# apache/bifromq

Hardware: AMD Instinct MI355X
Metric: publish-topic matches/sec (whole node) (higher is better)
Workload: dtype u32

## Files before the change

### bifromq_amd/csrc/bmq_build_core.h

```cpp
#pragma once
#include <sched.h>
#include <stdint.h>

#include "bmq_layout.h"

namespace bmq {

#if defined(__HIP_DEVICE_COMPILE__)
#define BMQ_MO_LOAD __ATOMIC_RELAXED
#define BMQ_MO_STORE __ATOMIC_RELAXED
#define BMQ_MO_RMW __ATOMIC_RELAXED
template <class T> BMQ_HD T atom_load(const T* p) { return __hip_atomic_load(p, __ATOMIC_RELAXED, __HIP_MEMORY_SCOPE_AGENT); }
template <class T> BMQ_HD void shared_store(T* p, T v) { __hip_atomic_store(p, v, __ATOMIC_RELAXED, __HIP_MEMORY_SCOPE_AGENT); }
template <class T> BMQ_HD T shared_load(const T* p) { return __hip_atomic_load(p, __ATOMIC_RELAXED, __HIP_MEMORY_SCOPE_AGENT); }
template <class T> BMQ_HD void atom_publish(T* p, T v) {
    asm volatile("s_waitcnt vmcnt(0)" ::: "memory");
    __hip_atomic_store(p, v, __ATOMIC_RELAXED, __HIP_MEMORY_SCOPE_AGENT);
}
template <class T> BMQ_HD T atom_cas(T* p, T expect, T desired) {
    __hip_atomic_compare_exchange_strong(p, &expect, desired, __ATOMIC_RELAXED, __ATOMIC_RELAXED, __HIP_MEMORY_SCOPE_AGENT);
    return expect;
}
template <class T> BMQ_HD T atom_add(T* p, T v) { return __hip_atomic_fetch_add(p, v, __ATOMIC_RELAXED, __HIP_MEMORY_SCOPE_AGENT); }
template <class T> BMQ_HD T atom_or(T* p, T v) { return __hip_atomic_fetch_or(p, v, __ATOMIC_RELAXED, __HIP_MEMORY_SCOPE_AGENT); }
// ... 181 lines not shown
}
BMQ_HD uint32_t tail_hash(const uint8_t* kp, unsigned long long beg, unsigned long long end) {
    uint32_t h = 0x811C9DC5u ^ (uint32_t)(end - beg);
    for (unsigned long long p = beg; p < end; p += 16) {
        uint32_t w[4];
        bytes_chunk16(kp, p, (uint32_t)(end - p < 16 ? end - p : 16), w);
        h = (h ^ w[0]) * 0x01000193u;
        h = (rotl32(h, 13) ^ w[1]) * 0x01000193u;
        h = (rotl32(h, 13) ^ w[2]) * 0x01000193u;
        h = (rotl32(h, 13) ^ w[3]) * 0x01000193u;
    }
    return mix32(h) | 1u;
}
BMQ_HD bool pool_bytes_equal(const uint8_t* kp, unsigned long long ao, unsigned long long bo, unsigned long long n) {
    for (unsigned long long i = 0; i < n; i += 16) {
        uint32_t x[4], y[4];
        const uint32_t m = (uint32_t)(n - i < 16 ? n - i : 16);
        bytes_chunk16(kp, ao + i, m, x);
        bytes_chunk16(kp, bo + i, m, y);
        if (((x[0] ^ y[0]) | (x[1] ^ y[1]) | (x[2] ^ y[2]) | (x[3] ^ y[3])) != 0) return false;
    }
    return true;
}
BMQ_HD bool bytes_equal(const uint8_t* a, unsigned long long ao, const uint8_t* b, unsigned long long bo, unsigned long long n) {
    for (unsigned long long i = 0; i < n; i++)
        if (a[ao + i] != b[bo + i]) return false;
    return true;
}
BMQ_HD int bytes_compare(const uint8_t* p, unsigned long long a, unsigned long long an, unsigned long long b, unsigned long long bn) {
    const unsigned long long m = an < bn ? an : bn;
    for (unsigned long long i = 0; i < m; i++) {
        const int d = (int)p[a + i] - (int)p[b + i];
        if (d) return d;
    }
    return an < bn ? -1 : (an > bn ? 1 : 0);
}

BMQ_HD uint32_t tenant_find(const TenantSlot* dir, uint32_t mask, const uint8_t* names, const uint8_t* kp, unsigned long long beg,
                            unsigned long long end) {
    const uint64_t h = tenant_hash_bytes(kp, beg, end);
    const uint32_t lo = (uint32_t)h, hi = (uint32_t)(h >> 32), len = (uint32_t)(end - beg);
    uint32_t d = (lo ^ hi) & mask;
    for (uint32_t probes = 0; probes <= mask; probes++) {
        const TenantSlot& t = dir[d];
        if (t.hash_lo == 0 && t.hash_hi == 0) return NONE;
        if (t.hash_lo == lo && t.hash_hi == hi && t.name_len == len && bytes_equal(names, t.name_off, kp, beg, len)) return d;
        d = (d + 1) & mask;
    }
    return NONE;
}

BMQ_HD uint32_t dict_intern(const DistIndexMut& ix, const LevelHash& h, uint32_t len, const uint32_t inl[4], const uint8_t* kp,
                            unsigned long long start, bool insert) {
    const uint32_t tag = level_hash_tag(h);
    uint32_t g = level_hash_slot(h, len) & ix.dict_group_mask;
    for (uint32_t jj = 0; jj < DICT_GROUP; jj++) {
        const DictSlot* s = ix.dict + DICT_GROUP * (size_t)g + jj;
        if (peek_load(&s->tag) != tag) continue;
        const uint32_t tok = peek_load(&s->token);
        if (tok == 0 || peek_load(&s->len) != len || peek_load(&s->inl[0]) != inl[0] || peek_load(&s->inl[1]) != inl[1] || peek_load(&s->inl[2]) != inl[2] ||
            peek_load(&s->inl[3]) != inl[3])
            continue;
        bool eq = true;
        if (len > 16) {
            const uint32_t po = peek_load(&s->pool_off);
            for (uint32_t i = 16; i < len && eq; i++) eq = peek_load(ix.dpool + po + i) == kp[start + i];
        }
        if (eq) return tok;
    }
    uint32_t j = 0, probes = 0, spins = 0;
    const uint32_t max_probes = insert && ix.dict_group_mask > 128u ? 128u : ix.dict_group_mask;
    for (;;) {
        if (probes > max_probes || spins > (1u << 22)) {
            atom_or(&ix.bc->err, probes > max_probes ? (uint32_t)ERR_DICT_FULL : (uint32_t)ERR_STUCK);
            return TOK_UNKNOWN;
        }
        DictSlot* s = ix.dict + DICT_GROUP * (size_t)g + j;
        uint32_t t = atom_load(&s->tag);
        if (t == 0) {
            if (!insert) return TOK_UNKNOWN;
            t = atom_cas(&s->tag, 0u, tag);
            if (t == 0) {
                uint32_t off = 0;
                if (len > 16) {
                    off = atom_add(&ix.bc->dpool_used, (len + 3u) & ~3u);
                    if ((unsigned long long)off + len > ix.dpool_cap) {
                        atom_or(&ix.bc->err, (uint32_t)ERR_DICT_FULL);
                        off = 0;
                    } else
                        for (uint32_t i = 0; i < len; i++) shared_store(ix.dpool + off + i, kp[start + i]);
                }
                shared_store(&s->len, len);
                shared_store(&s->pool_off, off);
                shared_store(&s->inl[0], inl[0]);
                shared_store(&s->inl[1], inl[1]);
                shared_store(&s->inl[2], inl[2]);
                shared_store(&s->inl[3], inl[3]);
                const uint32_t tok = TOK_FIRST + atom_add(&ix.bc->n_tokens, 1u);
                atom_publish(&s->token, tok);
                return tok;
            }
        }
        if (t == tag) {
            const uint32_t tok = atom_load(&s->token);
            if (tok == 0) {
                spin_pause(spins++);
                continue;
            }
            bool eq = shared_load(&s->len) == len && shared_load(&s->inl[0]) == inl[0] && shared_load(&s->inl[1]) == inl[1] &&
                      shared_load(&s->inl[2]) == inl[2] && shared_load(&s->inl[3]) == inl[3];
            if (eq && len > 16) {
                const uint32_t po = shared_load(&s->pool_off);
                for (uint32_t i = 16; i < len && eq; i++) eq = shared_load(ix.dpool + po + i) == kp[start + i];
            }
            if (eq) return tok;
        }
        if (++j == DICT_GROUP) {
            j = 0;
            g = (g + 1) & ix.dict_group_mask;
            probes++;
        }
    }
}

constexpr unsigned long long PARENT_IS_ROOT = ~0ull;
BMQ_HD uint32_t trie_child(const DistIndexMut& ix, TenantSlot* ten, uint32_t base, uint32_t buckets, uint32_t parent, unsigned long long parent_slot,
                           uint32_t token, bool insert, unsigned long long& slot_abs, bool& created) {
    created = false;
    const uint64_t key = (uint64_t)parent | ((uint64_t)token << 32);
    const bool root_plus = token == TOK_PLUS && parent_slot == PARENT_IS_ROOT;
    const bool try_beside = token == TOK_PLUS && parent_slot != PARENT_IS_ROOT;
    const unsigned long long beside_abs = parent_slot ^ 1ull;
    uint32_t phase = 0, spins = 0, bk = 0, j = 0, probes = 0;
    TrieSlot* wait = nullptr;
    unsigned long long wait_abs = 0;
    {
        auto peek = [&](unsigned long long abs) -> uint32_t {
            const TrieSlot* s = ix.trie + (size_t)abs;
            if (peek_load(reinterpret_cast<const uint64_t*>(s)) != key) return NONE;
            return peek_load(&s->node);
        };
        if (try_beside) {
            const uint32_t id = peek(beside_abs);
            if (id != NONE) {
                slot_abs = beside_abs;
                return id;
            }
        }
        if (!root_plus) {
            const unsigned long long home = (unsigned long long)base + 2ull * edge_bucket(parent, token, buckets);
            for (uint32_t jj = 0; jj < 2; jj++) {
                const uint32_t id = peek(home + jj);
                if (id != NONE) {
                    slot_abs = home + jj;
                    return id;
                }
            }
        }
    }
    for (;;) {
        if (spins > (1u << 22)) {
            atom_or(&ix.bc->err, (uint32_t)ERR_STUCK);
            return NONE;
// ... 566 lines not shown
            rec.parent = x.node;
            rec.token = TOK_TAIL;
            rec.own_begin = c.own_count != 0 ? c.own_begin : c.hash_begin;
            rec.own_count = c.own_count != 0 ? c.own_count : (c.hash_count | TAIL_HASH);
            rec.hash_begin = toks[0], rec.hash_count = toks[1], rec.node = toks[2], rec.lit_bloom = toks[3];
            ix.trie[g ^ 1u] = rec;
            return;
        }
        if (n != 1u || c.own_count != 0 || c.hash_count != 0) return;
        rel = tp.kid[r->nbase + c.node];
    }
}


BMQ_HD bool find_filter(const DistIndexMut& ix, const uint8_t* q, uint32_t tenant_len, uint32_t filter_len, IdSet& out) {
    out = IdSet{0, 0};
    const uint32_t d = tenant_find(ix.tenants, ix.tenant_mask, ix.tenant_names, q, 0, tenant_len);
    if (d == NONE) return false;
    TenantSlot* ten = ix.tenants + d;
    uint32_t node = 0;
    unsigned long long slot_abs = 0, pos = tenant_len;
    const unsigned long long end = (unsigned long long)tenant_len + filter_len;
    bool at_root = true;
    for (;;) {
        LevelHash h;
        uint32_t inl[4], len;
        const unsigned long long start = pos;
        scan_level_bytes<0x2F2F2F2Fu>(q, pos, end, h, inl, len);
        const bool last = pos >= end;
        if (level_is_hash(q, start, len, last)) {
            if (at_root) out = IdSet{ten->root_hash_begin, ten->root_hash_count};
            else out = IdSet{ix.trie[slot_abs].hash_begin, ix.trie[slot_abs].hash_count};
            return out.count() != 0;
        }
        const uint32_t tok = level_is_plus(q, start, len) ? TOK_PLUS : dict_intern(ix, h, len, inl, q, start, false);
        if (tok == TOK_UNKNOWN) return false;
        bool created;
        node = trie_child(ix, ten, ten->base, ten->buckets, node, at_root ? PARENT_IS_ROOT : slot_abs, tok, false, slot_abs, created);
        if (node == NONE) return false;
        at_root = false;
        if (last) break;
        pos++;
    }
    out = IdSet{ix.trie[slot_abs].own_begin, ix.trie[slot_abs].own_count};
    return out.count() != 0;
}

BMQ_HD void dict_rehash_one(const DictSlot* old, uint32_t i, const DistIndexMut& ix) {
    const DictSlot s = old[i];
    if (s.tag == 0) return;
    LevelHash h = level_hash_init();
    for (uint32_t o = 0; o < s.len; o += 4) {
        uint32_t w;
        if (s.len <= 16) w = s.inl[o >> 2];
        else {
            w = 0;
            for (uint32_t k = 0; k < 4 && o + k < s.len; k++) w |= (uint32_t)ix.dpool[s.pool_off + o + k] << (8 * k);
        }
        level_hash_word(h, w);
    }
    uint32_t g = level_hash_slot(h, s.len) & ix.dict_group_mask, j = 0;
    for (uint32_t probes = 0; probes <= ix.dict_group_mask;) {
        DictSlot* d = ix.dict + DICT_GROUP * (size_t)g + j;
        if (atom_cas(&d->tag, 0u, s.tag) == 0u) {
            d->len = s.len;
            d->pool_off = s.pool_off;
            d->inl[0] = s.inl[0];
            d->inl[1] = s.inl[1];
            d->inl[2] = s.inl[2];
            d->inl[3] = s.inl[3];
            d->token = s.token;
            return;
        }
        if (++j == DICT_GROUP) {
            j = 0;
            g = (g + 1) & ix.dict_group_mask;
            probes++;
        }
    }
    atom_or(&ix.bc->err, (uint32_t)ERR_DICT_FULL);
}

BMQ_HD void find_copy(const DistIndexMut& ix, const uint8_t* q, uint32_t tenant_len, uint32_t filter_len, uint32_t* out, uint32_t cap) {
    IdSet s;
    if (!find_filter(ix, q, tenant_len, filter_len, s)) {
        out[0] = 0;
        return;
    }
    const uint32_t n = s.count();
    out[0] = n;
    for (uint32_t m = 0; m < n && m < cap; m++) out[1 + m] = idset_at(ix, s, m);
}
BMQ_HD void gather_ref_one(const DistIndexMut& ix, const uint32_t* ids, uint32_t i, uint32_t id_end, unsigned long long* out) {
    const uint32_t id = ids[i];
    out[i] = id < id_end && id < ix.id_cap ? ix.kref[id] : 0ull;
}
BMQ_HD void gather_bytes_one(const DistIndexMut& ix, const unsigned long long* refs, const uint64_t* offs, uint32_t i, uint8_t* out) {
    const unsigned long long r = refs[i];
    const unsigned long long off = r & KREF_OFF_MASK, len = r >> KREF_LEN_SHIFT;
    for (unsigned long long k = 0; k < len; k++) out[offs[i] + k] = ix.kpool[off + k];
}

struct KeyBoundary {
    const uint8_t* start;
    const uint8_t* end;
    uint32_t start_len, end_len;
    uint32_t flags;
};
BMQ_HD int key_compare(const uint8_t* a, unsigned long long an, const uint8_t* b, unsigned long long bn) {
    const unsigned long long m = an < bn ? an : bn;
    unsigned long long p = 0;
    for (; p + 8 <= m; p += 8) {
        unsigned long long x, y;
        __builtin_memcpy(&x, a + p, 8);
        __builtin_memcpy(&y, b + p, 8);
        if (x != y) return __builtin_bswap64(x) < __builtin_bswap64(y) ? -1 : 1;
    }
    for (; p < m; p++)
        if (a[p] != b[p]) return a[p] < b[p] ? -1 : 1;
    return an < bn ? -1 : (an > bn ? 1 : 0);
}
BMQ_HD bool key_in_boundary(const uint8_t* kpool, unsigned long long ref, const KeyBoundary& b) {
    const uint8_t* k = kpool + (ref & KREF_OFF_MASK);
// ... 25 lines not shown
```

### bifromq_amd/csrc/bmq_dict.h

```cpp
#pragma once
#include <algorithm>
#include <cstring>
#include <string_view>
#include <vector>

#include "bmq_layout.h"

namespace bmq {

inline LevelHash hash_level(std::string_view s) {
    LevelHash h = level_hash_init();
    for (size_t i = 0; i < s.size(); i += 4) {
        uint32_t w = 0;
        for (size_t k = 0; k < 4 && i + k < s.size(); k++) w |= (uint32_t)(uint8_t)s[i + k] << (8 * k);
        level_hash_word(h, w);
    }
    return h;
}

inline uint32_t pow2_at_least(uint64_t v) {
    uint32_t p = 64;
    while (p < v && p < 0x80000000u) p <<= 1;
    return p;
}

struct HostDict {
    struct Entry {
        std::string_view s;
        uint32_t slot_hash, tag;
    };
    std::vector<Entry> entries;
    std::vector<uint32_t> table;
    uint32_t mask = 0;
    HostDict() { table.assign(1024, 0); mask = 1023; }
    void grow() {
        std::vector<uint32_t> nt(table.size() * 2, 0);
        const uint32_t nm = (uint32_t)nt.size() - 1;
        for (uint32_t t = 0; t < entries.size(); t++) {
            uint32_t i = entries[t].slot_hash & nm;
            while (nt[i]) i = (i + 1) & nm;
            nt[i] = t + TOK_FIRST;
        }
        table.swap(nt);
        mask = nm;
    }
    uint32_t find(std::string_view s) const {
        const LevelHash h = hash_level(s);
        const uint32_t sh = level_hash_slot(h, (uint32_t)s.size()), tag = level_hash_tag(h);
        uint32_t i = sh & mask;
        while (table[i]) {
            const Entry& e = entries[table[i] - TOK_FIRST];
            if (e.tag == tag && e.s == s) return table[i];
            i = (i + 1) & mask;
        }
        return TOK_UNKNOWN;
    }
    uint32_t intern(std::string_view s) {
        const LevelHash h = hash_level(s);
        const uint32_t sh = level_hash_slot(h, (uint32_t)s.size()), tag = level_hash_tag(h);
        uint32_t i = sh & mask;
        while (table[i]) {
            const Entry& e = entries[table[i] - TOK_FIRST];
            if (e.tag == tag && e.s == s) return table[i];
            i = (i + 1) & mask;
        }
        entries.push_back({s, sh, tag});
        const uint32_t tok = (uint32_t)entries.size() - 1 + TOK_FIRST;
        table[i] = tok;
        if (entries.size() * 2 > table.size()) grow();
        return tok;
    }
};


inline void flatten_dict(const HostDict& dict_h, std::vector<DictSlot>& dict, std::vector<uint8_t>& pool) {
    const uint32_t dslots = pow2_at_least(std::max<uint64_t>(8, (uint64_t)dict_h.entries.size() * 4));
    const uint32_t gmask = dslots / DICT_GROUP - 1;
    dict.assign(dslots, DictSlot{0, 0, 0, 0, {0, 0, 0, 0}});
    pool.clear();
    for (size_t t = 0; t < dict_h.entries.size(); t++) {
        const auto& e = dict_h.entries[t];
        uint32_t g = e.slot_hash & gmask, s = NONE;
        for (;;) {
            for (uint32_t j = 0; j < DICT_GROUP && s == NONE; j++)
                if (!dict[DICT_GROUP * g + j].tag) s = DICT_GROUP * g + j;
            if (s != NONE) break;
            g = (g + 1) & gmask;
        }
        DictSlot& d = dict[s];
        d.tag = e.tag;
        d.token = (uint32_t)t + TOK_FIRST;
        d.len = (uint32_t)e.s.size();
        for (size_t i = 0; i < e.s.size() && i < 16; i++) d.inl[i >> 2] |= (uint32_t)(uint8_t)e.s[i] << (8 * (i & 3));
        if (e.s.size() > 16) {
            d.pool_off = (uint32_t)pool.size();
            pool.insert(pool.end(), e.s.begin(), e.s.end());
        }
    }
    while (pool.size() % 16 || pool.empty()) pool.push_back(0);
}

inline uint32_t dict_find(const std::vector<DictSlot>& dict, const std::vector<uint8_t>& pool, std::string_view level) {
    if (dict.empty()) return TOK_UNKNOWN;
    const LevelHash h = hash_level(level);
    const uint32_t gmask = (uint32_t)dict.size() / DICT_GROUP - 1, tag = level_hash_tag(h);
    uint32_t g = level_hash_slot(h, (uint32_t)level.size()) & gmask;
    for (;;) {
        bool group_full = true;
        for (uint32_t j = 0; j < DICT_GROUP; j++) {
            const DictSlot& d = dict[DICT_GROUP * g + j];
            if (!d.tag) {
                group_full = false;
                continue;
            }
            if (d.tag == tag && d.len == level.size()) {
                bool eq = true;
                for (size_t i = 0; i < level.size() && i < 16 && eq; i++)
                    eq = ((d.inl[i >> 2] >> (8 * (i & 3))) & 0xFF) == (uint8_t)level[i];
                if (eq && level.size() > 16) eq = memcmp(pool.data() + d.pool_off, level.data(), level.size()) == 0;
                if (eq) return d.token;
            }
        }
        if (!group_full) return TOK_UNKNOWN;
        g = (g + 1) & gmask;
    }
}

}
```

### bifromq_amd/csrc/bmq_dist_kernels.h

```cpp
#pragma once
#ifndef BMQ_WAVE_EMU
#include <hip/hip_runtime.h>
#endif

#include <type_traits>

#include "bmq_layout.h"
#include "bmq_batch_args.h"

namespace bmq {

#ifndef BMQ_WAVE_EMU
__device__ __forceinline__ void wave_sync() {
    __builtin_amdgcn_fence(__ATOMIC_RELEASE, "wavefront");
    __builtin_amdgcn_wave_barrier();
    __builtin_amdgcn_fence(__ATOMIC_ACQUIRE, "wavefront");
}
__device__ __forceinline__ uint32_t rank_below(unsigned long long mask) {
    return __builtin_amdgcn_mbcnt_hi((uint32_t)(mask >> 32), __builtin_amdgcn_mbcnt_lo((uint32_t)mask, 0u));
}
#endif
__device__ __forceinline__ uint32_t wave_excl_scan(uint32_t v, uint32_t lane, uint32_t& total) {
    uint32_t inc = v;
#pragma unroll
    for (int d = 1; d < 64; d <<= 1) {
        const uint32_t o = __shfl_up(inc, d);
        if (lane >= (uint32_t)d) inc += o;
    }
    total = __shfl(inc, 63);
    return inc - v;
}
__device__ __forceinline__ unsigned long long wave_sum_u64(unsigned long long v) {
#pragma unroll
    for (int d = 32; d >= 1; d >>= 1) v += __shfl_xor(v, d);
    return v;
}

__device__ __forceinline__ TrieSlot unpack_slot(const uint4& a, const uint4& b) {
    TrieSlot s;
    s.parent = a.x; s.token = a.y; s.own_begin = a.z; s.own_count = a.w;
    s.hash_begin = b.x; s.hash_count = b.y; s.node = b.z; s.lit_bloom = b.w;
    return s;
}
struct Line64 {
    uint4 a0, a1, b0, b1;
};
static_assert(DICT_GROUP == 2, "a dictionary group is one Line64");
#ifndef BMQ_WAVE_EMU
__device__ __forceinline__ void load_line64(const void* p, Line64& r) {
    asm volatile("global_load_dwordx4 %0, %4, off\n\t"
                 "global_load_dwordx4 %1, %4, off offset:16\n\t"
                 "global_load_dwordx4 %2, %4, off offset:32\n\t"
                 "global_load_dwordx4 %3, %4, off offset:48\n\t"
                 "s_waitcnt vmcnt(0)"
                 : "=&v"(r.a0), "=&v"(r.a1), "=&v"(r.b0), "=&v"(r.b1)
                 : "v"(p));
}
__device__ __forceinline__ void load_line64_s(const void* sbase, uint32_t voff, Line64& r) {
    asm volatile("global_load_dwordx4 %0, %4, %5\n\t"
                 "global_load_dwordx4 %1, %4, %5 offset:16\n\t"
                 "global_load_dwordx4 %2, %4, %5 offset:32\n\t"
                 "global_load_dwordx4 %3, %4, %5 offset:48\n\t"
                 "s_waitcnt vmcnt(0)"
                 : "=&v"(r.a0), "=&v"(r.a1), "=&v"(r.b0), "=&v"(r.b1)
                 : "v"(voff), "s"(sbase));
}
#else
inline void load_line64(const void* p, Line64& r) { memcpy(&r, p, 64); }
inline void load_line64_s(const void* sbase, uint32_t voff, Line64& r) { memcpy(&r, reinterpret_cast<const uint8_t*>(sbase) + voff, 64); }
#endif
template <class ByteAt>
__device__ __forceinline__ uint32_t dict_lookup(const DistIndexView& ix, const LevelHash& h, uint32_t len,
                                                const uint32_t inl[4], uint32_t start, ByteAt&& byte_at) {
    const uint32_t tag = level_hash_tag(h);
    uint32_t g = level_hash_slot(h, len) & ix.dict_group_mask;
    auto tail_eq = [&](uint32_t pool_off) {
        bool eq = true;
        for (uint32_t i = 16; i < len && eq; i++) eq = ix.pool[pool_off + i] == byte_at(start + i);
        return eq;
    };
    for (uint32_t probes = 0; probes <= ix.dict_group_mask; probes++) {
        Line64 ln;
        load_line64(ix.dict + DICT_GROUP * (size_t)g, ln);
        const bool h0 = ln.a0.x == tag && ln.a0.z == len && ln.a1.x == inl[0] && ln.a1.y == inl[1] && ln.a1.z == inl[2] &&
                        ln.a1.w == inl[3];
        const bool h1 = ln.b0.x == tag && ln.b0.z == len && ln.b1.x == inl[0] && ln.b1.y == inl[1] && ln.b1.z == inl[2] &&
                        ln.b1.w == inl[3];
        if (h0 && (len <= 16 || tail_eq(ln.a0.w))) return ln.a0.y;
        if (h1 && (len <= 16 || tail_eq(ln.b0.w))) return ln.b0.y;
        if (ln.a0.x == 0 || ln.b0.x == 0) return TOK_UNKNOWN;
        g = (g + 1) & ix.dict_group_mask;
    }
    return TOK_UNKNOWN;
}

#ifndef BMQ_WAVE_EMU
__device__ __forceinline__ void load_slot32(const void* p, uint4& a, uint4& b) {
    asm volatile("global_load_dwordx4 %0, %2, off\n\t"
                 "global_load_dwordx4 %1, %2, off offset:16\n\t"
                 "s_waitcnt vmcnt(0)"
                 : "=&v"(a), "=&v"(b)
                 : "v"(p));
}
#else
inline void load_slot32(const void* p, uint4& a, uint4& b) {
    memcpy(&a, p, 16);
    memcpy(&b, reinterpret_cast<const uint8_t*>(p) + 16, 16);
}
#endif
template <class ByteAt>
__device__ __forceinline__ uint32_t dict_lookup_by_slot(const DistIndexView& ix, const LevelHash& h, uint32_t len, const uint32_t inl[4], uint32_t start,
                                                        ByteAt&& byte_at) {
    const uint32_t tag = level_hash_tag(h);
    uint32_t g = level_hash_slot(h, len) & ix.dict_group_mask;
    auto tail_eq = [&](uint32_t pool_off) {
        bool eq = true;
        for (uint32_t i = 16; i < len && eq; i++) eq = ix.pool[pool_off + i] == byte_at(start + i);
        return eq;
    };
    for (uint32_t probes = 0; probes <= ix.dict_group_mask; probes++) {
        const DictSlot* grp = ix.dict + DICT_GROUP * (size_t)g;
#pragma unroll
        for (uint32_t k = 0; k < DICT_GROUP; k++) {
            uint4 hd, in;
            load_slot32(grp + k, hd, in);
            if (hd.x == tag && hd.z == len && in.x == inl[0] && in.y == inl[1] && in.z == inl[2] && in.w == inl[3] && (len <= 16 || tail_eq(hd.w))) return hd.y;
            if (hd.x == 0) return TOK_UNKNOWN;
        }
        g = (g + 1) & ix.dict_group_mask;
    }
    return TOK_UNKNOWN;
}

template <class WordAt>
__device__ __forceinline__ void scan_level(uint32_t& pos, uint32_t end, bool split, WordAt&& word_at, LevelHash& h,
                                           uint32_t inl[4], uint32_t& len, bool& last) {
    h = level_hash_init();
    inl[0] = inl[1] = inl[2] = inl[3] = 0;
    len = 0;
    for (;;) {
        const uint32_t remaining = end - pos;
        if (remaining == 0) break;
        const uint32_t w = word_at(pos);
        uint32_t nb = 4;
        if (split) {
            const uint32_t x = w ^ 0x2F2F2F2Fu;
            const uint32_t z = (x - 0x01010101u) & ~x & 0x80808080u;
            if (z) nb = (uint32_t)(__ffs((int)z) - 1) >> 3;
        }
        nb = min(nb, remaining);
        if (nb) {
            const uint32_t wm = nb == 4 ? w : (w & ((1u << (8u * nb)) - 1u));
            level_hash_word(h, wm);
            if (len < 16) inl[len >> 2] = wm;
            len += nb;
            pos += nb;
        }
        if (nb < 4) break;
    }
    if (pos < end) {
        pos++;
        last = false;
    } else {
        last = true;
    }
}

__device__ __forceinline__ uint32_t global_word_at(const uint8_t* base, uint32_t p) {
    const uint32_t* a = reinterpret_cast<const uint32_t*>(base + (p & ~3u));
    return __builtin_amdgcn_alignbyte(a[1], a[0], p & 3u);
}

constexpr TenantSlot EMPTY_TENANT{0, 0, 0, 0, 0, 1, 0, 0, 0, 0, 0, 0, {0, 0, 0}, NONE};
__device__ __forceinline__ bool tenant_known(const TenantSlot& t) { return (t.hash_lo | t.hash_hi) != 0; }

__global__ __launch_bounds__(64) void k_reset(Counters* ctr, SubAlloc* subs, unsigned long long* super_sums, uint32_t n_super) {
    const uint32_t i = blockIdx.x * 64 + threadIdx.x;
    if (i < sizeof(Counters) / 8) reinterpret_cast<unsigned long long*>(ctr)[i] = 0ull;
    if (i < sizeof(SubAlloc) * 2 * N_SUB / 8) reinterpret_cast<unsigned long long*>(subs)[i] = 0ull;
// ... 380 lines not shown
```

### bifromq_amd/csrc/bmq_layout.h

```cpp
#pragma once
#include <stdint.h>
#include <stdlib.h>

#ifndef BMQ_EXPERIMENTS
#define BMQ_EXPERIMENTS 0
#endif
inline const char* bmq_env(const char* name) { return BMQ_EXPERIMENTS ? getenv(name) : nullptr; }

#if defined(__HIP__)
#include <hip/hip_runtime.h>
#define BMQ_HD __host__ __device__ inline __attribute__((always_inline))
#else
#define BMQ_HD inline
#endif

namespace bmq {

constexpr uint32_t NONE = 0xFFFFFFFFu;
constexpr uint32_t TOK_UNKNOWN = 0;
constexpr uint32_t TOK_PLUS = 1;
constexpr uint32_t TOK_FIRST = 2;
constexpr uint32_t TOK_TOMB = 0xFFFFFFFDu;
constexpr uint32_t TOK_TAIL = 0xFFFFFFFEu;
constexpr uint32_t TAIL_K = 4;
constexpr uint32_t TAIL_HASH = 0x40000000u;
#ifndef BMQ_FAST_LEVELS
#define BMQ_FAST_LEVELS 16
#endif
constexpr int FAST_LEVELS = BMQ_FAST_LEVELS;
constexpr uint32_t RANGE_INDIRECT = 0x80000000u;
constexpr uint32_t BLOOM_PLUS = 0x80000000u;
constexpr uint64_t EDGE_EMPTY = 0x00000000FFFFFFFFull;

struct alignas(32) TrieSlot {
    uint32_t parent;
    uint32_t token;
    uint32_t own_begin;
    uint32_t own_count;
    uint32_t hash_begin;
    uint32_t hash_count;
    uint32_t node;
    uint32_t lit_bloom;
};
static_assert(sizeof(TrieSlot) == 32, "TrieSlot must be 32 bytes");
BMQ_HD bool slot_is_node(const TrieSlot& s) { return s.parent != NONE && s.token < TOK_TOMB; }

struct alignas(64) TenantSlot {
    uint32_t hash_lo, hash_hi;
    uint32_t name_off, name_len;
    uint32_t base;
    uint32_t buckets;
    uint32_t n_nodes;
    uint32_t n_routes;
    uint32_t root_hash_begin, root_hash_count;
    uint32_t root_lit_bloom;
    uint32_t pending;
    uint32_t name12[3];
    uint32_t root_plus;
};
static_assert(sizeof(TenantSlot) == 64, "TenantSlot must be 64 bytes");

constexpr uint32_t DICT_GROUP = 2;
struct alignas(32) DictSlot {
    uint32_t tag;
    uint32_t token;
    uint32_t len;
    uint32_t pool_off;
    uint32_t inl[4];
};
static_assert(sizeof(DictSlot) == 32, "DictSlot must be 32 bytes");

struct LevelHash {
    uint32_t h1, h2;
};
BMQ_HD uint32_t rotl32(uint32_t x, uint32_t r) { return (x << r) | (x >> (32u - r)); }
BMQ_HD LevelHash level_hash_init() { return {0x811C9DC5u, 0x9747B28Cu}; }
BMQ_HD void level_hash_word(LevelHash& h, uint32_t w) {
    h.h1 = rotl32(h.h1, 5) ^ w;
    h.h1 += h.h1 << 3;
    h.h2 = rotl32(h.h2, 11) + w;
    h.h2 ^= h.h2 >> 7;
}
BMQ_HD uint32_t mix32(uint32_t x) {
    x ^= x >> 16;
    x *= 0x7FEB352Du;
    x ^= x >> 15;
    x *= 0x846CA68Bu;
    x ^= x >> 16;
    return x;
}
BMQ_HD uint32_t level_hash_slot(const LevelHash& h, uint32_t len) { return mix32(h.h1 ^ (len * 0x85EBCA6Bu)); }
BMQ_HD uint32_t level_hash_tag(const LevelHash& h) {
    uint32_t x = h.h2 ^ (h.h1 >> 3);
    x ^= x >> 15;
    x *= 0x2C1B3C6Du;
    x ^= x >> 13;
    return x | 1u;
}

BMQ_HD uint32_t edge_bucket(uint32_t parent, uint32_t token, uint32_t buckets) {
    uint32_t h = (parent ^ rotl32(token, 16)) * 0x9E3779B1u;
    h ^= h >> 15;
    h *= 0x85EBCA77u;
    h ^= h >> 13;
    return (uint32_t)(((uint64_t)h * buckets) >> 32);
}
BMQ_HD uint32_t bloom_bit(uint32_t token) {
    const uint32_t b = (token ^ (token >> 5) ^ (token >> 11)) & 31u;
    return b - (b == 31u ? 1u : 0u);
}
constexpr uint32_t FILTER_MUL = 0x9E3779B1u;
constexpr uint32_t FILTER_NONE = 0xFFFFFFFFu;
BMQ_HD uint32_t filter_bit_own(uint32_t token) { return (token * FILTER_MUL) >> 27; }
BMQ_HD uint32_t filter_bit_hash(uint32_t token) { return ((token * FILTER_MUL) >> 22) & 31u; }
BMQ_HD uint32_t filter_word(uint32_t begin, uint32_t count) { return count == 0 ? begin : FILTER_NONE; }
BMQ_HD uint64_t tenant_hash_step(uint64_t h, uint32_t byte) { return (h ^ byte) * 0x100000001B3ull; }
constexpr uint64_t TENANT_HASH_INIT = 0xCBF29CE484222325ull;
BMQ_HD uint64_t tenant_hash_final(uint64_t h) {
    h ^= h >> 33;
    h *= 0xFF51AFD7ED558CCDull;
    h ^= h >> 29;
    return h ? h : 1ull;
}

struct DistIndexView {
    const TrieSlot* trie;
    const TenantSlot* tenants;
    uint32_t tenant_mask;
    uint32_t filter_off;
    const uint8_t* tenant_names;
    const DictSlot* dict;
    uint32_t dict_group_mask;
    const uint8_t* pool;
    const uint32_t* route_pos;
};

struct MatchRange {
    uint32_t begin, count;
};

}
```

### bifromq_amd/csrc/bmq_retain_core.h

```cpp
#pragma once
#include <stdint.h>

#include "bmq_build_core.h"
#include "bmq_key_core.h"
#include "bmq_retain.h"

namespace bmq {

#if defined(__HIP_DEVICE_COMPILE__)
template <class T> BMQ_HD T atom_max(T* p, T v) { return __hip_atomic_fetch_max(p, v, __ATOMIC_RELAXED, __HIP_MEMORY_SCOPE_AGENT); }
template <class T> BMQ_HD T atom_and(T* p, T v) { return __hip_atomic_fetch_and(p, v, __ATOMIC_RELAXED, __HIP_MEMORY_SCOPE_AGENT); }
template <class T> BMQ_HD T atom_xchg(T* p, T v) { return __hip_atomic_exchange(p, v, __ATOMIC_RELAXED, __HIP_MEMORY_SCOPE_AGENT); }
BMQ_HD void atom_drain() { asm volatile("s_waitcnt vmcnt(0)" ::: "memory"); }
#else
template <class T> BMQ_HD T atom_max(T* p, T v) {
    T cur = __atomic_load_n(p, __ATOMIC_ACQUIRE);
    while (cur < v && !__atomic_compare_exchange_n(p, &cur, v, false, __ATOMIC_ACQ_REL, __ATOMIC_ACQUIRE)) {
    }
    return cur;
}
template <class T> BMQ_HD T atom_and(T* p, T v) { return __atomic_fetch_and(p, v, __ATOMIC_ACQ_REL); }
template <class T> BMQ_HD T atom_xchg(T* p, T v) { return __atomic_exchange_n(p, v, __ATOMIC_ACQ_REL); }
BMQ_HD void atom_drain() {}
#endif

constexpr uint32_t RT_OVERLAY = 0x80000000u;
constexpr uint32_t ID_SYS = 0x80000000u;
enum : uint32_t { RERR_NODES = 1u, RERR_POOL = 2u, RERR_IDS = 4u, RERR_STUCK = 8u, RERR_BAD_OP = 16u };

struct RetainCounters {
    uint32_t ov_nodes;
    uint32_t opool_used;
    uint32_t next_id;
    uint32_t err;
    uint32_t went_live[N_CTR_LANES], went_dead[N_CTR_LANES];
    uint32_t base_went_live[N_CTR_LANES], base_went_dead[N_CTR_LANES];
};

struct RetainMut {
    RetainIndexView base;
    uint32_t base_n;
    ONode* onodes;
    uint32_t ov_cap;
    uint32_t* oedges;
    uint32_t oedge_mask;
    uint8_t* opool;
    uint32_t opool_cap;
    unsigned long long* expire_at;
    unsigned long long* ts;
    uint32_t* expiry;
    uint32_t* id_node;
    uint32_t* id_tnode;
    uint32_t id_cap;
    unsigned long long* dead_bits;
    uint32_t* dead_rank;
    unsigned long long* last_op;
    RetainCounters* ctr;
};

struct RetainOps {
    const uint8_t* tenants;
    const uint32_t* tenant_off;
    uint32_t n_tenants;
    const uint32_t* op_tenant;
    const uint8_t* topics;
    const uint32_t* topic_off;
    const uint8_t* op;
    const unsigned long long* ts;
    const uint32_t* expiry;
    uint32_t n;
    unsigned long long seq;
    uint32_t* target;
    uint32_t* out_ids;
};

BMQ_HD uint32_t rdict_find(const RetainIndexView& ix, const LevelHash& h, uint32_t len, const uint32_t inl[4], const uint8_t* bytes,
                           unsigned long long start) {
    const uint32_t tag = level_hash_tag(h);
    uint32_t g = level_hash_slot(h, len) & ix.dict_group_mask;
    for (uint32_t probes = 0; probes <= ix.dict_group_mask; probes++) {
        bool free_slot = false;
        for (uint32_t j = 0; j < DICT_GROUP; j++) {
            const DictSlot& s = ix.dict[DICT_GROUP * (size_t)g + j];
            if (s.tag == 0) {
                free_slot = true;
                continue;
            }
            if (s.tag != tag || s.len != len || s.inl[0] != inl[0] || s.inl[1] != inl[1] || s.inl[2] != inl[2] || s.inl[3] != inl[3]) continue;
            bool eq = true;
            for (uint32_t i = 16; i < len && eq; i++) eq = ix.pool[s.pool_off + i] == bytes[start + i];
            if (eq) return s.token;
        }
        if (free_slot) return TOK_UNKNOWN;
        g = (g + 1) & ix.dict_group_mask;
    }
    return TOK_UNKNOWN;
}
BMQ_HD uint32_t redge_find(const RetainIndexView& ix, uint32_t edge_base, uint32_t mask, uint32_t parent, uint32_t token) {
    uint32_t bk = redge_bucket(parent, token, mask);
    for (uint32_t probes = 0; probes <= mask; probes++) {
        bool free_slot = false;
        for (uint32_t j = 0; j < 4; j++) {
            const REdge& e = ix.edges[edge_base + 4 * (size_t)bk + j];
            if (e.parent == parent && e.token == token) return e.child & ~RE_OVERFLOW;
            free_slot = free_slot || e.parent == NONE;
        }
        if (free_slot) return NONE;
        bk = (bk + 1) & mask;
    }
    return NONE;
}
BMQ_HD const RTenantSlot* rtenant_find(const RetainIndexView& ix, uint32_t token) {
    uint32_t d = tenant_hash(token) & ix.tenant_mask;
    for (uint32_t probes = 0; probes <= ix.tenant_mask; probes++) {
        const RTenantSlot& t = ix.tenants[d];
        if (t.token == token) return &t;
        if (t.token == 0) return nullptr;
        d = (d + 1) & ix.tenant_mask;
    }
    return nullptr;
}
struct LevelScan {
    LevelHash h;
    uint32_t inl[4];
    uint32_t len;
    unsigned long long start;
    bool more;
};
BMQ_HD void next_level(const uint8_t* bytes, unsigned long long& pos, unsigned long long end, LevelScan& lv) {
    lv.start = pos;
    scan_level_bytes<0x2F2F2F2Fu>(bytes, pos, end, lv.h, lv.inl, lv.len);
    lv.more = pos < end;
    if (lv.more) pos++;
}
BMQ_HD uint32_t base_find(const RetainIndexView& ix, uint32_t base_n, const uint8_t* tenants, unsigned long long tb, unsigned long long te,
                          const uint8_t* topics, unsigned long long pb, unsigned long long pe) {
    if (base_n == 0) return NONE;
    LevelScan lv;
    unsigned long long pos = tb;
    lv.start = pos;
    scan_level_bytes<0u>(tenants, pos, te, lv.h, lv.inl, lv.len);
// ... 438 lines not shown
```

### bifromq_amd/csrc/bmq_walk_kernel.h

```cpp
#pragma once

namespace bmq {

constexpr uint32_t WALK_MAX_TENANTS = 4;
__device__ __forceinline__ uint32_t walk_meta(uint32_t tl, uint32_t tokpos, uint32_t rem) { return tl | (tokpos << 6) | (rem << 16); }
constexpr uint32_t WALK_META_CHILD = 64u - 65536u;

#define BMQ_WALK_GEOM_DEFAULT 512, 176, 152
#define BMQ_WALK_GEOM_SMALLEST 192, 128, 128
constexpr uint32_t WALK_QC_DEFAULT = 176, WALK_PC_DEFAULT = 152, WALK_QC_SMALLEST = 128, WALK_PC_SMALLEST = 128;

template <int TC, int QC, int PC, bool MIXED> struct WalkLds {
    static constexpr uint32_t TOK = 0;
    static constexpr uint32_t STK = TOK + TC * 4;
    static constexpr uint32_t PRG = STK + QC * 8;
    static constexpr uint32_t PTP = PRG + PC * 8;
    static constexpr uint32_t VIS = PTP + PC;
    static constexpr uint32_t REG = VIS + 64 * 4;
    static constexpr uint32_t BYTES = (REG + (MIXED ? 64 * 8 : 0) + 15) & ~15u;
    static constexpr uint32_t STAGE = BYTES - STK;
    static constexpr uint32_t ALLOC = (BYTES + 511) & ~511u;
#ifndef BMQ_WALK_MAX_WAVES
#define BMQ_WALK_MAX_WAVES 8
#endif
// ... 65 lines not shown
    const bool staged = (s_end - a0) + 32u <= G::STAGE;
    if (staged) {
        uint4* dst = reinterpret_cast<uint4*>(stk);
        const uint4* src = reinterpret_cast<const uint4*>(a.topics + a0);
        const uint32_t n16 = (s_end - a0 + 15) >> 4;
        for (uint32_t o = lane; o < n16; o += 64) dst[o] = src[o];
    }
    uint32_t nlev = 0, pos = 0, end = 0, ti = 0xFFFFFFFFu;
    if (valid) {
        pos = a.topic_off[t];
        end = a.topic_off[t + 1];
        ti = a.topic_tenant[t];
    }
    const bool asked = ti < a.n_tenants && (a.rep == nullptr || a.rep[t] == t);
    wave_sync();
    const uint8_t* lbytes = reinterpret_cast<const uint8_t*>(stk);
    const uint32_t* lwords = reinterpret_cast<const uint32_t*>(stk);
    const uint8_t* gbytes = a.topics;
    if (asked) {
        uint32_t cnt = 1;
        for (uint32_t p = pos & ~3u; p < end; p += 4) {
            const uint32_t w = staged ? lwords[(p - a0) >> 2] : *reinterpret_cast<const uint32_t*>(gbytes + p);
            const uint32_t x = w ^ 0x2F2F2F2Fu;
            uint32_t z = ~(((x & 0x7F7F7F7Fu) + 0x7F7F7F7Fu) | x | 0x7F7F7F7Fu);
            if (p < pos) z &= 0xFFFFFFFFu << (8u * (pos - p));
            if (p + 4 > end) z &= 0xFFFFFFFFu >> (8u * (p + 4 - end));
            cnt += (uint32_t)__popc(z);
        }
        nlev = cnt;
    }
    const bool deep = nlev > (uint32_t)FAST_LEVELS;
    const bool sys = asked && end > pos && (staged ? (uint32_t)lbytes[pos - a0] : (uint32_t)gbytes[pos]) == '$';
    const unsigned long long clkA = dbg_clock(dbg_w);
    uint32_t tok_base = 0;
    auto tokenise = [&](bool mine, bool from_lds) {
        auto byte_at = [&](uint32_t i) -> uint32_t { return from_lds ? (uint32_t)lbytes[i - a0] : (uint32_t)gbytes[i]; };
        auto word_at = [&](uint32_t i) -> uint32_t {
            if (!from_lds) return global_word_at(gbytes, i);
            const uint32_t rel = i - a0;
            return __builtin_amdgcn_alignbyte(lwords[(rel >> 2) + 1], lwords[rel >> 2], rel & 3u);
        };
        bool more = mine;
        uint32_t p = pos;
        for (uint32_t l = 0; ballot64(more) != 0; l++) {
            LevelHash h = level_hash_init();
            uint32_t inl[4] = {0, 0, 0, 0}, len = 0;
            const uint32_t start = p;
            const bool now = more;
            if (more) {
                bool last;
                scan_level(p, end, true, word_at, h, inl, len, last);
                more = !last;
            }
            const uint32_t tok = now ? (BMQ_DBG(a, 128u) ? dict_lookup(a.ix, h, len, inl, start, byte_at) : dict_lookup_by_slot(a.ix, h, len, inl, start, byte_at))
                                     : TOK_UNKNOWN;
            if (now) tokens[tok_base + l] = tok;
        }
    };

    uint32_t tail = 0, pcount = 0, rounds = 0, items = 0;
    const uint32_t f_off = a.ix.filter_off;
    uint32_t fl_base = 0, fl_len = 0;
    uint32_t qs_base = 0, qs_len = 0;
    auto spill_alloc = [&](const BatchArgs& c, uint32_t ln, uint32_t n, uint32_t& base) -> bool {
        unsigned long long sb = 0;
        uint32_t ok = 1;
        if (ln == 0) ok = pair_alloc(c.subs + N_SUB, c.spill_cap, blk, n + 1, sb) ? 1u : 0u;
        const uint32_t lo = sgpr((uint32_t)sb), hi = sgpr((uint32_t)(sb >> 32));
        const bool fits = sgpr(ok) != 0 && hi == 0 && lo + n + 1 < 0xFFFFFFFFu && lo + n + 1 > lo;
        if (!fits && ln == 0) atomicOr(&c.ctr->status, ST_NEED_SPILL);
        base = lo;
        return fits;
    };
    const unsigned long long clk1 = dbg_clock(dbg_w);
    auto sink = [&](uint32_t own_begin, uint32_t own_count , uint32_t hash_begin, uint32_t hash_count ,
                    uint32_t lit , uint32_t bloom , uint32_t child,
                    uint32_t cmeta , uint32_t tl, uint32_t ln ) {
        const bool emit_own = own_count != 0, emit_hash = hash_count != 0, push_l = lit != 0, push_h = (int32_t)bloom < 0;
        const unsigned long long m_own = ballot64(emit_own), m_hash = ballot64(emit_hash);
        const unsigned long long m_l = ballot64(push_l), m_h = ballot64(push_h);
        if ((m_own | m_hash) != 0) {
            const uint32_t n_own = (uint32_t)__popcll(m_own), n_emit = n_own + (uint32_t)__popcll(m_hash);
            if (__builtin_expect(pcount + n_emit > (uint32_t)PC, 0)) {
                const BatchArgs& c = a;
                BMQ_WALK_COV(flushes);
                uint32_t cb;
                if (spill_alloc(c, ln, pcount, cb)) {
                    if (ln == 0) c.spill[cb] = make_uint4(fl_base, fl_len, 0u, 0u);
                    for (uint32_t i = ln; i < pcount; i += 64) c.spill[cb + 1 + i] = make_uint4(p_rng[i].x, p_rng[i].y, p_topic[i], 0u);
                    fl_base = cb;
                    fl_len = pcount;
                }
                pcount = 0;
                wave_sync();
            }
            if (emit_own) {
                const uint32_t p = pcount + rank_below(m_own);
                p_rng[p] = make_uint2(own_begin, own_count);
                p_topic[p] = (uint8_t)tl;
            }
            if (emit_hash) {
                const uint32_t p = pcount + n_own + rank_below(m_hash);
                p_rng[p] = make_uint2(hash_begin, hash_count);
                p_topic[p] = (uint8_t)tl;
            }
            pcount += n_emit;
        }
// ... 382 lines not shown
```

Baseline: 3.988 billion.

## Reorder DictSlot so short levels match with one 16-byte load

DictSlot is reordered so the tag, token and first 8 inline bytes sit in the first 16 bytes, and the level length is folded into the tag's low byte. When no lane in the wave has a level longer than 8 bytes, the walk kernel probes the dictionary with a single dwordx4 load per slot instead of two. The goal is less memory traffic and latency per dictionary probe for short topic levels. The cost is a wave-uniform branch, and every host and device reader and writer of the dict layout has to be updated consistently.

```diff
diff --git a/bifromq_amd/csrc/bmq_build_core.h b/bifromq_amd/csrc/bmq_build_core.h
--- a/bifromq_amd/csrc/bmq_build_core.h
+++ b/bifromq_amd/csrc/bmq_build_core.h
@@ -257,14 +257,14 @@
 
 BMQ_HD uint32_t dict_intern(const DistIndexMut& ix, const LevelHash& h, uint32_t len, const uint32_t inl[4], const uint8_t* kp,
                             unsigned long long start, bool insert) {
-    const uint32_t tag = level_hash_tag(h);
+    const uint32_t tag = dict_tag(h, len);
     uint32_t g = level_hash_slot(h, len) & ix.dict_group_mask;
     for (uint32_t jj = 0; jj < DICT_GROUP; jj++) {
         const DictSlot* s = ix.dict + DICT_GROUP * (size_t)g + jj;
         if (peek_load(&s->tag) != tag) continue;
         const uint32_t tok = peek_load(&s->token);
-        if (tok == 0 || peek_load(&s->len) != len || peek_load(&s->inl[0]) != inl[0] || peek_load(&s->inl[1]) != inl[1] || peek_load(&s->inl[2]) != inl[2] ||
-            peek_load(&s->inl[3]) != inl[3])
+        if (tok == 0 || peek_load(&s->len) != len || peek_load(&s->inl[0]) != inl[0] || peek_load(&s->inl[1]) != inl[1] || peek_load(&s->inl_hi[0]) != inl[2] ||
+            peek_load(&s->inl_hi[1]) != inl[3])
             continue;
         bool eq = true;
         if (len > 16) {
@@ -299,8 +299,8 @@
                 shared_store(&s->pool_off, off);
                 shared_store(&s->inl[0], inl[0]);
                 shared_store(&s->inl[1], inl[1]);
-                shared_store(&s->inl[2], inl[2]);
-                shared_store(&s->inl[3], inl[3]);
+                shared_store(&s->inl_hi[0], inl[2]);
+                shared_store(&s->inl_hi[1], inl[3]);
                 const uint32_t tok = TOK_FIRST + atom_add(&ix.bc->n_tokens, 1u);
                 atom_publish(&s->token, tok);
                 return tok;
@@ -313,7 +313,7 @@
                 continue;
             }
             bool eq = shared_load(&s->len) == len && shared_load(&s->inl[0]) == inl[0] && shared_load(&s->inl[1]) == inl[1] &&
-                      shared_load(&s->inl[2]) == inl[2] && shared_load(&s->inl[3]) == inl[3];
+                      shared_load(&s->inl_hi[0]) == inl[2] && shared_load(&s->inl_hi[1]) == inl[3];
             if (eq && len > 16) {
                 const uint32_t po = shared_load(&s->pool_off);
                 for (uint32_t i = 16; i < len && eq; i++) eq = shared_load(ix.dpool + po + i) == kp[start + i];
@@ -986,7 +986,7 @@
     LevelHash h = level_hash_init();
     for (uint32_t o = 0; o < s.len; o += 4) {
         uint32_t w;
-        if (s.len <= 16) w = s.inl[o >> 2];
+        if (s.len <= 16) w = dict_inl(s, o >> 2);
         else {
             w = 0;
             for (uint32_t k = 0; k < 4 && o + k < s.len; k++) w |= (uint32_t)ix.dpool[s.pool_off + o + k] << (8 * k);
@@ -1001,8 +1001,8 @@
             d->pool_off = s.pool_off;
             d->inl[0] = s.inl[0];
             d->inl[1] = s.inl[1];
-            d->inl[2] = s.inl[2];
-            d->inl[3] = s.inl[3];
+            d->inl_hi[0] = s.inl_hi[0];
+            d->inl_hi[1] = s.inl_hi[1];
             d->token = s.token;
             return;
         }
diff --git a/bifromq_amd/csrc/bmq_dict.h b/bifromq_amd/csrc/bmq_dict.h
--- a/bifromq_amd/csrc/bmq_dict.h
+++ b/bifromq_amd/csrc/bmq_dict.h
@@ -46,7 +46,7 @@
     }
     uint32_t find(std::string_view s) const {
         const LevelHash h = hash_level(s);
-        const uint32_t sh = level_hash_slot(h, (uint32_t)s.size()), tag = level_hash_tag(h);
+        const uint32_t sh = level_hash_slot(h, (uint32_t)s.size()), tag = dict_tag(h, (uint32_t)s.size());
         uint32_t i = sh & mask;
         while (table[i]) {
             const Entry& e = entries[table[i] - TOK_FIRST];
@@ -57,7 +57,7 @@
     }
     uint32_t intern(std::string_view s) {
         const LevelHash h = hash_level(s);
-        const uint32_t sh = level_hash_slot(h, (uint32_t)s.size()), tag = level_hash_tag(h);
+        const uint32_t sh = level_hash_slot(h, (uint32_t)s.size()), tag = dict_tag(h, (uint32_t)s.size());
         uint32_t i = sh & mask;
         while (table[i]) {
             const Entry& e = entries[table[i] - TOK_FIRST];
@@ -76,7 +76,7 @@
 inline void flatten_dict(const HostDict& dict_h, std::vector<DictSlot>& dict, std::vector<uint8_t>& pool) {
     const uint32_t dslots = pow2_at_least(std::max<uint64_t>(8, (uint64_t)dict_h.entries.size() * 4));
     const uint32_t gmask = dslots / DICT_GROUP - 1;
-    dict.assign(dslots, DictSlot{0, 0, 0, 0, {0, 0, 0, 0}});
+    dict.assign(dslots, DictSlot{0, 0, {0, 0}, 0, 0, {0, 0}});
     pool.clear();
     for (size_t t = 0; t < dict_h.entries.size(); t++) {
         const auto& e = dict_h.entries[t];
@@ -91,7 +91,7 @@
         d.tag = e.tag;
         d.token = (uint32_t)t + TOK_FIRST;
         d.len = (uint32_t)e.s.size();
-        for (size_t i = 0; i < e.s.size() && i < 16; i++) d.inl[i >> 2] |= (uint32_t)(uint8_t)e.s[i] << (8 * (i & 3));
+        for (size_t i = 0; i < e.s.size() && i < 16; i++) dict_inl(d, (uint32_t)i >> 2) |= (uint32_t)(uint8_t)e.s[i] << (8 * (i & 3));
         if (e.s.size() > 16) {
             d.pool_off = (uint32_t)pool.size();
             pool.insert(pool.end(), e.s.begin(), e.s.end());
@@ -103,7 +103,7 @@
 inline uint32_t dict_find(const std::vector<DictSlot>& dict, const std::vector<uint8_t>& pool, std::string_view level) {
     if (dict.empty()) return TOK_UNKNOWN;
     const LevelHash h = hash_level(level);
-    const uint32_t gmask = (uint32_t)dict.size() / DICT_GROUP - 1, tag = level_hash_tag(h);
+    const uint32_t gmask = (uint32_t)dict.size() / DICT_GROUP - 1, tag = dict_tag(h, (uint32_t)level.size());
     uint32_t g = level_hash_slot(h, (uint32_t)level.size()) & gmask;
     for (;;) {
         bool group_full = true;
@@ -116,7 +116,7 @@
             if (d.tag == tag && d.len == level.size()) {
                 bool eq = true;
                 for (size_t i = 0; i < level.size() && i < 16 && eq; i++)
-                    eq = ((d.inl[i >> 2] >> (8 * (i & 3))) & 0xFF) == (uint8_t)level[i];
+                    eq = ((dict_inl(d, (uint32_t)i >> 2) >> (8 * (i & 3))) & 0xFF) == (uint8_t)level[i];
                 if (eq && level.size() > 16) eq = memcmp(pool.data() + d.pool_off, level.data(), level.size()) == 0;
                 if (eq) return d.token;
             }
diff --git a/bifromq_amd/csrc/bmq_dist_kernels.h b/bifromq_amd/csrc/bmq_dist_kernels.h
--- a/bifromq_amd/csrc/bmq_dist_kernels.h
+++ b/bifromq_amd/csrc/bmq_dist_kernels.h
@@ -72,7 +72,7 @@
 template <class ByteAt>
 __device__ __forceinline__ uint32_t dict_lookup(const DistIndexView& ix, const LevelHash& h, uint32_t len,
                                                 const uint32_t inl[4], uint32_t start, ByteAt&& byte_at) {
-    const uint32_t tag = level_hash_tag(h);
+    const uint32_t tag = dict_tag(h, len);
     uint32_t g = level_hash_slot(h, len) & ix.dict_group_mask;
     auto tail_eq = [&](uint32_t pool_off) {
         bool eq = true;
@@ -82,12 +82,12 @@
     for (uint32_t probes = 0; probes <= ix.dict_group_mask; probes++) {
         Line64 ln;
         load_line64(ix.dict + DICT_GROUP * (size_t)g, ln);
-        const bool h0 = ln.a0.x == tag && ln.a0.z == len && ln.a1.x == inl[0] && ln.a1.y == inl[1] && ln.a1.z == inl[2] &&
+        const bool h0 = ln.a0.x == tag && ln.a1.x == len && ln.a0.z == inl[0] && ln.a0.w == inl[1] && ln.a1.z == inl[2] &&
                         ln.a1.w == inl[3];
-        const bool h1 = ln.b0.x == tag && ln.b0.z == len && ln.b1.x == inl[0] && ln.b1.y == inl[1] && ln.b1.z == inl[2] &&
+        const bool h1 = ln.b0.x == tag && ln.b1.x == len && ln.b0.z == inl[0] && ln.b0.w == inl[1] && ln.b1.z == inl[2] &&
                         ln.b1.w == inl[3];
-        if (h0 && (len <= 16 || tail_eq(ln.a0.w))) return ln.a0.y;
-        if (h1 && (len <= 16 || tail_eq(ln.b0.w))) return ln.b0.y;
+        if (h0 && (len <= 16 || tail_eq(ln.a1.y))) return ln.a0.y;
+        if (h1 && (len <= 16 || tail_eq(ln.b1.y))) return ln.b0.y;
         if (ln.a0.x == 0 || ln.b0.x == 0) return TOK_UNKNOWN;
         g = (g + 1) & ix.dict_group_mask;
     }
@@ -95,6 +95,12 @@
 }
 
 #ifndef BMQ_WAVE_EMU
+__device__ __forceinline__ void load_slot16(const void* p, uint4& a) {
+    asm volatile("global_load_dwordx4 %0, %1, off\n\t"
+                 "s_waitcnt vmcnt(0)"
+                 : "=&v"(a)
+                 : "v"(p));
+}
 __device__ __forceinline__ void load_slot32(const void* p, uint4& a, uint4& b) {
     asm volatile("global_load_dwordx4 %0, %2, off\n\t"
                  "global_load_dwordx4 %1, %2, off offset:16\n\t"
@@ -103,16 +109,39 @@
                  : "v"(p));
 }
 #else
+struct DictLoadCount {
+    unsigned long long first = 0, second = 0;
+};
+inline DictLoadCount dict_loads;
+inline void load_slot16(const void* p, uint4& a) {
+    memcpy(&a, p, 16);
+    dict_loads.first++;
+}
 inline void load_slot32(const void* p, uint4& a, uint4& b) {
     memcpy(&a, p, 16);
     memcpy(&b, reinterpret_cast<const uint8_t*>(p) + 16, 16);
+    dict_loads.first++, dict_loads.second++;
 }
 #endif
 template <class ByteAt>
 __device__ __forceinline__ uint32_t dict_lookup_by_slot(const DistIndexView& ix, const LevelHash& h, uint32_t len, const uint32_t inl[4], uint32_t start,
-                                                        ByteAt&& byte_at) {
-    const uint32_t tag = level_hash_tag(h);
+                                                        bool wide, ByteAt&& byte_at) {
+    const uint32_t tag = dict_tag(h, len);
     uint32_t g = level_hash_slot(h, len) & ix.dict_group_mask;
+    if (!wide) {
+        for (uint32_t probes = 0; probes <= ix.dict_group_mask; probes++) {
+            const DictSlot* grp = ix.dict + DICT_GROUP * (size_t)g;
+#pragma unroll
+            for (uint32_t k = 0; k < DICT_GROUP; k++) {
+                uint4 hd;
+                load_slot16(grp + k, hd);
+                if (hd.x == tag && hd.z == inl[0] && hd.w == inl[1]) return hd.y;
+                if (hd.x == 0) return TOK_UNKNOWN;
+            }
+            g = (g + 1) & ix.dict_group_mask;
+        }
+        return TOK_UNKNOWN;
+    }
     auto tail_eq = [&](uint32_t pool_off) {
         bool eq = true;
         for (uint32_t i = 16; i < len && eq; i++) eq = ix.pool[pool_off + i] == byte_at(start + i);
@@ -124,7 +153,7 @@
         for (uint32_t k = 0; k < DICT_GROUP; k++) {
             uint4 hd, in;
             load_slot32(grp + k, hd, in);
-            if (hd.x == tag && hd.z == len && in.x == inl[0] && in.y == inl[1] && in.z == inl[2] && in.w == inl[3] && (len <= 16 || tail_eq(hd.w))) return hd.y;
+            if (hd.x == tag && in.x == len && hd.z == inl[0] && hd.w == inl[1] && in.z == inl[2] && in.w == inl[3] && (len <= 16 || tail_eq(in.y))) return hd.y;
             if (hd.x == 0) return TOK_UNKNOWN;
         }
         g = (g + 1) & ix.dict_group_mask;
diff --git a/bifromq_amd/csrc/bmq_layout.h b/bifromq_amd/csrc/bmq_layout.h
--- a/bifromq_amd/csrc/bmq_layout.h
+++ b/bifromq_amd/csrc/bmq_layout.h
@@ -64,11 +64,15 @@
 struct alignas(32) DictSlot {
     uint32_t tag;
     uint32_t token;
+    uint32_t inl[2];
     uint32_t len;
     uint32_t pool_off;
-    uint32_t inl[4];
+    uint32_t inl_hi[2];
 };
 static_assert(sizeof(DictSlot) == 32, "DictSlot must be 32 bytes");
+constexpr uint32_t DICT_SHORT = 8;
+BMQ_HD uint32_t& dict_inl(DictSlot& s, uint32_t k) { return k < 2 ? s.inl[k] : s.inl_hi[k - 2]; }
+BMQ_HD const uint32_t& dict_inl(const DictSlot& s, uint32_t k) { return k < 2 ? s.inl[k] : s.inl_hi[k - 2]; }
 
 struct LevelHash {
     uint32_t h1, h2;
@@ -97,6 +101,7 @@
     x ^= x >> 13;
     return x | 1u;
 }
+BMQ_HD uint32_t dict_tag(const LevelHash& h, uint32_t len) { return (level_hash_tag(h) & 0xFFFFFF00u) | 0x100u | (len < 255u ? len : 255u); }
 
 BMQ_HD uint32_t edge_bucket(uint32_t parent, uint32_t token, uint32_t buckets) {
     uint32_t h = (parent ^ rotl32(token, 16)) * 0x9E3779B1u;
diff --git a/bifromq_amd/csrc/bmq_retain_core.h b/bifromq_amd/csrc/bmq_retain_core.h
--- a/bifromq_amd/csrc/bmq_retain_core.h
+++ b/bifromq_amd/csrc/bmq_retain_core.h
@@ -76,7 +76,7 @@
 
 BMQ_HD uint32_t rdict_find(const RetainIndexView& ix, const LevelHash& h, uint32_t len, const uint32_t inl[4], const uint8_t* bytes,
                            unsigned long long start) {
-    const uint32_t tag = level_hash_tag(h);
+    const uint32_t tag = dict_tag(h, len);
     uint32_t g = level_hash_slot(h, len) & ix.dict_group_mask;
     for (uint32_t probes = 0; probes <= ix.dict_group_mask; probes++) {
         bool free_slot = false;
@@ -86,7 +86,7 @@
                 free_slot = true;
                 continue;
             }
-            if (s.tag != tag || s.len != len || s.inl[0] != inl[0] || s.inl[1] != inl[1] || s.inl[2] != inl[2] || s.inl[3] != inl[3]) continue;
+            if (s.tag != tag || s.len != len || s.inl[0] != inl[0] || s.inl[1] != inl[1] || s.inl_hi[0] != inl[2] || s.inl_hi[1] != inl[3]) continue;
             bool eq = true;
             for (uint32_t i = 16; i < len && eq; i++) eq = ix.pool[s.pool_off + i] == bytes[start + i];
             if (eq) return s.token;
diff --git a/bifromq_amd/csrc/bmq_walk_kernel.h b/bifromq_amd/csrc/bmq_walk_kernel.h
--- a/bifromq_amd/csrc/bmq_walk_kernel.h
+++ b/bifromq_amd/csrc/bmq_walk_kernel.h
@@ -141,7 +141,8 @@
                 scan_level(p, end, true, word_at, h, inl, len, last);
                 more = !last;
             }
-            const uint32_t tok = now ? (BMQ_DBG(a, 128u) ? dict_lookup(a.ix, h, len, inl, start, byte_at) : dict_lookup_by_slot(a.ix, h, len, inl, start, byte_at))
+            const bool wide = ballot64(len > DICT_SHORT) != 0;
+            const uint32_t tok = now ? (BMQ_DBG(a, 128u) ? dict_lookup(a.ix, h, len, inl, start, byte_at) : dict_lookup_by_slot(a.ix, h, len, inl, start, wide, byte_at))
                                      : TOK_UNKNOWN;
             if (now) tokens[tok_base + l] = tok;
         }
```

Result: no change. 4.049 billion, median of 3 (+1.5%).
